# KyleJHarper/tyche

Measured on AMD Instinct MI355X. Metric: GiB/s device-resident LZ4 compress+decompress, 1M×16KiB pages, 1/2/4/8 GPU, higher is better.
Workload: dtype u8

## Files before the change

### tyche_amd/csrc/lz4_encode.hip

```cpp
#include <hip/hip_runtime.h>

#define TYCHE_PHASES_OWNER
#define TYCHE_HASH_LOG 10
#ifndef TYCHE_PARSE_LATCH
#define TYCHE_PARSE_LATCH 1
#endif

#include <algorithm>
#include <cstdlib>

#include "engine.h"
#include "lds_io.h"
#include "lz_parse.h"

namespace tyche {

namespace {

using lzp::kWave;
using lzp::kHashSize;
constexpr uint32_t kPad = 64;
constexpr uint32_t kPrefetchVec = 16;

struct SeqFields {
    uint32_t lit, lext, anchor, off, mc, token, total;
};

__device__ __forceinline__ uint32_t seq_byte(const SeqFields &f, const uint8_t *in, uint32_t rel) {
    const uint32_t lb = 1 + f.lext, ob = lb + f.lit;
    const uint32_t li = f.anchor + min(rel - lb, f.lit - 1u);
    const uint32_t litb = in[rel >= lb && f.lit ? li : 0u];
    const uint32_t ext = rel == f.lext ? (f.lit - 15u) % 255u : 255u;
    const uint32_t mext = rel == f.total - 1u ? (f.mc - 15u) % 255u : 255u;
    uint32_t v = mext;
    v = rel == ob + 1u ? f.off >> 8 : v;
    v = rel == ob ? f.off & 0xFFu : v;
    v = rel < ob ? litb : v;
    v = rel <= f.lext ? ext : v;
    v = rel == 0u ? f.token : v;
    return v;
}


__device__ bool emit_records(const uint2 *rec, uint32_t n, uint32_t anchor, const uint8_t *in, uint8_t *dst,
                             uint32_t &op, uint32_t cap, uint8_t *map, uint4 *fld, uint32_t lane) {
    const bool is_sel = lane < n;
    const uint2 r = rec[is_sel ? lane : 0];
    const uint2 rp = rec[lane > 0 && is_sel ? lane - 1 : 0];
    const uint32_t pos = r.x & 0xFFFFu, cand = r.x >> 16, len = r.y & 0xFFFFu, back = lzp::back_at(in, pos, cand);
    const uint32_t prev_end = lane == 0 ? anchor : (rp.x & 0xFFFFu) + (rp.y & 0xFFFFu);
    SeqFields f{};
    uint32_t enc = 0;
    if (is_sel) {
        const uint32_t k = min(min(back, pos - prev_end), cand);
        f.anchor = prev_end;
        f.lit = pos - k - prev_end;
        f.lext = f.lit >= 15 ? (f.lit - 15) / 255 + 1 : 0;
        f.off = pos - cand;
        f.mc = len + k - kMinMatch;
        const uint32_t mext = f.mc >= 15 ? (f.mc - 15) / 255 + 1 : 0;
        f.token = (min(f.lit, 15u) << 4) | min(f.mc, 15u);
        f.total = 1 + f.lext + f.lit + 2 + mext;
        enc = f.total;
    }
    const int32_t incl = wave_incl_sum((int32_t)enc);
    const uint32_t eo = (uint32_t)incl - enc;
    const uint32_t et = rdlane((uint32_t)incl, 63);
    if (op + et > cap) return false;
    if (is_sel) fld[lane] = make_uint4(f.lit | (f.lext << 16), f.anchor | (f.off << 16), f.mc | (f.total << 16),
                                       eo | (f.token << 16));
    uint32_t *map32 = (uint32_t *)map;
    for (uint32_t j0 = 0; j0 < ((TYCHE_EABLATE & 1) ? 0u : et); j0 += 4u * kWave) {
        const uint64_t before = __ballot(is_sel && eo < j0);
        const int32_t owner0 = before ? 63 - (int32_t)__builtin_clzll(before) : 0;
        map32[lane] = 0xFFFFFFFFu;
        __builtin_amdgcn_wave_barrier();
        if (is_sel && eo >= j0 && eo < j0 + 4u * kWave) map[eo - j0] = (uint8_t)lane;
        __builtin_amdgcn_wave_barrier();
        const uint32_t m = map32[lane];
        int32_t last = -1;
#pragma unroll
        for (int t = 0; t < 4; t++) {
            const uint32_t st = (m >> (8 * t)) & 0xFFu;
            if (st != 0xFFu) last = (int32_t)st;
        }
        const int32_t incl_max = wave_incl_max(last);
        int32_t cur = (int32_t)__shfl(incl_max, (int)(lane ? lane - 1u : 0u));
        cur = max(lane ? cur : -1, owner0);
        const uint32_t jb = j0 + 4u * lane;
        uint32_t word = 0, prev_o = 0xFFFFFFFFu;
        uint4 g = make_uint4(0, 0, 0, 0);
#pragma unroll
        for (int t = 0; t < 4; t++) {
            const uint32_t st = (m >> (8 * t)) & 0xFFu;
            if (st != 0xFFu) cur = (int32_t)st;
            if (jb + (uint32_t)t < et) {
                if ((uint32_t)cur != prev_o) {
                    g = fld[cur];
                    prev_o = (uint32_t)cur;
                }
                SeqFields q;
                q.lit = g.x & 0xFFFFu;
                q.lext = g.x >> 16;
                q.anchor = g.y & 0xFFFFu;
                q.off = g.y >> 16;
                q.mc = g.z & 0xFFFFu;
                q.total = g.z >> 16;
                q.token = g.w >> 16;
                word |= seq_byte(q, in, jb + (uint32_t)t - (g.w & 0xFFFFu)) << (8 * t);
            }
        }
        if (jb + 4u <= et) {
            store_u32_unaligned(dst + op + jb, word);
        } else {
#pragma unroll
            for (int t = 0; t < 4; t++)
                if (jb + (uint32_t)t < et) dst[op + jb + (uint32_t)t] = (uint8_t)(word >> (8 * t));
        }
        __builtin_amdgcn_wave_barrier();
    }
    op += et;
    return true;
}

constexpr uint32_t kOutRing = 512;
constexpr uint32_t kFlushStep = 4u * kWave;
static_assert(kOutRing % kFlushStep == 0 && (kOutRing & (kOutRing - 1)) == 0, "ring");
static_assert(kOutRing + 64u * 8u == 1024u, "emit_records' fields fit the records and the ring");
constexpr uint32_t kLitLane = 8;
struct OutRing {
    uint32_t head, pend;
};

__device__ __forceinline__ void out_flush_steps(const uint8_t *ring, OutRing &r, uint8_t *dst, uint32_t &op,
                                                uint32_t lane) {
    while (r.pend >= kFlushStep) {
        const uint8_t *src = ring + ((r.head + 4u * lane) & (kOutRing - 1));
        store_u32_unaligned(dst + op + 4u * lane, *(const uint32_t *)src);
        op += kFlushStep;
        r.head = (r.head + kFlushStep) & (kOutRing - 1);
        r.pend -= kFlushStep;
    }
}

__device__ __forceinline__ void out_flush_all(const uint8_t *ring, OutRing &r, uint8_t *dst, uint32_t &op,
                                              uint32_t lane) {
    out_flush_steps(ring, r, dst, op, lane);
    for (uint32_t j = 4 * lane; j < r.pend; j += 4 * kWave) {
        const uint32_t w = *(const uint32_t *)(ring + ((r.head + j) & (kOutRing - 1)));
        if (j + 4 <= r.pend) {
            store_u32_unaligned(dst + op + j, w);
        } else {
            for (uint32_t t = 0; j + t < r.pend; t++) dst[op + j + t] = (uint8_t)(w >> (8 * t));
        }
    }
    op += r.pend;
    r.head = 0;
    r.pend = 0;
    __builtin_amdgcn_wave_barrier();
}

__device__ __forceinline__ bool emit_staged(const uint2 *rec, uint32_t n, uint32_t anchor, const uint8_t *in, uint8_t *dst,
                            uint32_t &op, uint32_t cap, uint8_t *ring, OutRing &r, uint8_t *map, uint32_t lane) {
#if defined(TYCHE_PHASES)
    const bool sp_rec = blockIdx.x % 64u == 0u && lane == 0u;
    uint32_t sp_t = (uint32_t)__builtin_amdgcn_s_memtime();
#define SINK_PHASE(i) do { const uint32_t t_ = (uint32_t)__builtin_amdgcn_s_memtime(); \
                           if (sp_rec) atomicAdd(&lzp::g_phase[i], (unsigned long long)(t_ - sp_t)); sp_t = t_; } while (0)
#else
#define SINK_PHASE(i) do {} while (0)
#endif
    const bool is_sel = lane < n;
    const uint2 rc = rec[is_sel ? lane : 0];
    const uint2 rp = rec[lane > 0 && is_sel ? lane - 1 : 0];
    const uint32_t pos = rc.x & 0xFFFFu, cand = rc.x >> 16, len = rc.y & 0xFFFFu, back = lzp::back_at(in, pos, cand);
    const uint32_t prev_end = lane == 0 ? anchor : (rp.x & 0xFFFFu) + (rp.y & 0xFFFFu);
    const uint32_t k = min(min(back, pos - prev_end), cand);
    const uint32_t lstart = prev_end;
    const uint32_t lit = is_sel ? pos - k - prev_end : 0u;
    const uint32_t lext = lit >= 15 ? (lit - 15) / 255 + 1 : 0;
    const uint32_t off = pos - cand;
    const uint32_t mc = len + k - kMinMatch;
    const uint32_t mext = mc >= 15 ? (mc - 15) / 255 + 1 : 0;
    const uint32_t token = (min(lit, 15u) << 4) | min(mc, 15u);
    const uint32_t enc = is_sel ? 1 + lext + lit + 2 + mext : 0u;
    const int32_t incl = wave_incl_sum((int32_t)enc);
    const uint32_t eo = (uint32_t)incl - enc;
    const uint32_t et = rdlane((uint32_t)incl, 63);
    if (op + r.pend + et > cap) return false;
    if (r.pend + et > kOutRing) {
        out_flush_all(ring, r, dst, op, lane);
        uint4 *fld = (uint4 *)(ring + kOutRing - 1024u);
        return emit_records(rec, n, anchor, in, dst, op, cap, map, fld, lane);
    }
    SINK_PHASE(11);
    constexpr uint32_t m = kOutRing - 1;
    const uint32_t q_lit = r.head + r.pend + eo + 1 + lext;
    if (is_sel) {
        uint32_t q = r.head + r.pend + eo;
        ring[q & m] = (uint8_t)token;
        q++;
        for (uint32_t t = 0; t < lext; t++) ring[(q + t) & m] = (uint8_t)(t + 1 == lext ? (lit - 15) % 255 : 255);
        const uint32_t ls = min(lit, kLitLane);
        static_assert(kLitLane == 8, "two gathered dwords");
        const uint32_t ib = (uint32_t)(uintptr_t)in & 3u;
        const uint32_t *A = (const uint32_t *)(in - ib);
        const uint32_t q0 = lstart + ib, i0 = q0 >> 2, sh = q0 & 3u;
        const uint32_t d0 = A[i0], d1 = A[i0 + 1], d2 = A[i0 + 2];
        const uint32_t w0 = __builtin_amdgcn_alignbyte(d1, d0, sh), w1 = __builtin_amdgcn_alignbyte(d2, d1, sh);
#pragma unroll
        for (uint32_t t = 0; t < 8; t++) {
            uint8_t *bp = t < ls ? ring + ((q_lit + t) & m) : map;
            *bp = (uint8_t)((t < 4 ? w0 : w1) >> (8 * (t & 3u)));
        }
        q = q_lit + lit;
        ring[q & m] = (uint8_t)off;
        ring[(q + 1) & m] = (uint8_t)(off >> 8);
        q += 2;
        for (uint32_t t = 0; t < mext; t++) ring[(q + t) & m] = (uint8_t)(t + 1 == mext ? (mc - 15) % 255 : 255);
    }
    SINK_PHASE(12);
    uint64_t longm = __ballot(is_sel && lit > kLitLane);
    while (longm) {
        const uint32_t k = (uint32_t)__builtin_ctzll(longm);
        longm &= longm - 1;
        const uint32_t kl = rdlane(lit, k) - kLitLane, kq = rdlane(q_lit, k) + kLitLane, ks = rdlane(lstart, k) + kLitLane;
        for (uint32_t i = lane; i < kl; i += kWave) ring[(kq + i) & m] = in[ks + i];
    }
    __builtin_amdgcn_wave_barrier();
    SINK_PHASE(13);
    r.pend += et;
    out_flush_steps(ring, r, dst, op, lane);
    __builtin_amdgcn_wave_barrier();
    SINK_PHASE(14);
#if defined(TYCHE_PHASES)
    if (sp_rec) atomicAdd(&lzp::g_phase[15], 1ull);
#endif
    return true;
}
#undef SINK_PHASE

__device__ __noinline__ bool emit_staged_call(const uint2 *rec, uint32_t n, uint32_t anchor, const uint8_t *in, uint8_t *dst,
                                              uint32_t &op, uint32_t cap, uint8_t *ring, OutRing &r, uint8_t *map,
                                              uint32_t lane) {
    return emit_staged(rec, n, anchor, in, dst, op, cap, ring, r, map, lane);
}

__device__ __forceinline__ bool emit_sink_n(const uint2 *rec, uint32_t n, uint32_t anchor, const uint8_t *in, uint8_t *dst,
                                            uint32_t &op, uint32_t cap, uint8_t *ring, OutRing &r, uint8_t *map,
                                            uint32_t lane) {
    return emit_staged(rec, n, anchor, in, dst, op, cap, ring, r, map, lane);
}

__device__ int32_t encode_page(const uint8_t *in, uint32_t L, uint16_t *table, uint8_t *map, uint2 *rec,
                               uint4 *fld, uint8_t *dst, uint32_t cap, uint32_t lane) {
    uint32_t op = 0;
    OutRing r{0u, 0u};
    uint8_t *ring = (uint8_t *)fld;
    auto sink = [&](const uint2 *rr, uint32_t n, uint32_t anchor) -> bool {
        return emit_staged_call(rr, n, anchor, in, dst, op, cap, ring, r, map, lane);
    };
    const uint32_t anchor = lzp::parse_page(in, L, table, rec, lane, sink);
    if (anchor == 0xFFFFFFFFu) return 0;
    out_flush_all(ring, r, dst, op, lane);
    const uint32_t lit = L - anchor;
    const uint32_t lext = lit >= 15 ? (lit - 15) / 255 + 1 : 0;
    const uint32_t total = 1 + lext + lit;
    if (op + total > cap) return 0;
    for (uint32_t j = lane; j < total; j += kWave) {
        uint32_t v;
        if (j == 0) v = min(lit, 15u) << 4;
        else if (j <= lext) v = j == lext ? (lit - 15) % 255 : 255;
        else v = in[anchor + j - 1 - lext];
        dst[op + j] = (uint8_t)v;
    }
    return (int32_t)(op + total);
}

constexpr uint32_t kSplitMin = 12288;
constexpr uint32_t kSplitAt = 36;
static_assert(kSplitAt >= 32 && kSplitAt < 64, "B's half must fit its scratch (sized for L / 2 + 64)");
constexpr uint32_t kSplitPrefetch = 8;
struct SplitHdr {
    uint32_t next_lo, next_hi, next2_lo, next2_hi;
    uint32_t len_a;
    uint32_t len_b;
    uint32_t has_first;
    int32_t result;
    uint2 first;
    uint32_t pad[6];
};
static_assert(sizeof(SplitHdr) == 64, "split header");
__device__ __forceinline__ void seed_table(const uint8_t *in, uint16_t *table, uint32_t from, uint32_t to,
                                           uint32_t lane) {
    const uint32_t ib = (uint32_t)(uintptr_t)in & 3u;
    const uint32_t la = lzp::lds_addr(in - ib) + ((lane + ib) & ~3u), ls = (lane + ib) & 3u;
    const uint32_t tbase = rfl(lzp::lds_addr(table));
    auto slot = [&](uint32_t w) { return (lzp::lds_u16_t *)(uintptr_t)lzp::slot_addr(tbase, lzp::hash4(w)); };
    uint32_t blk = from;
    for (; blk + 4u * kWave <= to; blk += 4u * kWave) {
        const lzp::lds_u32_t *P = (const lzp::lds_u32_t *)(uintptr_t)(la + blk);
        uint32_t w[4];
#pragma unroll
        for (uint32_t u = 0; u < 4u; u++) w[u] = lzp::word_at(P[16u * u], P[16u * u + 1u], ls);
#pragma unroll
        for (uint32_t u = 0; u < 4u; u++) {
            *slot(w[u]) = (uint16_t)(blk + kWave * u + lane);
            __builtin_amdgcn_wave_barrier();
        }
    }
    for (; blk < to; blk += kWave) {
        const lzp::lds_u32_t *P = (const lzp::lds_u32_t *)(uintptr_t)(la + blk);
        *slot(lzp::word_at(P[0], P[1], ls)) = (uint16_t)(blk + lane);
        __builtin_amdgcn_wave_barrier();
    }
}

constexpr size_t kWaveRegion = kHashSize * sizeof(uint16_t) + 4 * kWave + kWave * sizeof(uint2) + kOutRing;
constexpr size_t kSplitStage = sizeof(SplitHdr) + 2 * kWaveRegion;

__device__ bool write_last_literals(const uint8_t *in, uint32_t anchor, uint32_t L, uint8_t *dst, uint32_t &op,
                                    uint32_t cap, uint32_t lane) {
    const uint32_t lit = L - anchor;
    const uint32_t lext = lit >= 15 ? (lit - 15) / 255 + 1 : 0;
    const uint32_t total = 1 + lext + lit;
    if (op + total > cap) return false;
    for (uint32_t j = lane; j < total; j += kWave) {
        uint32_t v;
        if (j == 0) v = min(lit, 15u) << 4;
        else if (j <= lext) v = j == lext ? (lit - 15) % 255 : 255;
        else v = in[anchor + j - 1 - lext];
        dst[op + j] = (uint8_t)v;
    }
    op += total;
    return true;
}

__device__ __forceinline__ bool emit_joint(uint2 first, uint32_t prev_end, const uint8_t *in, uint8_t *dst, uint32_t &op,
                                           uint32_t cap, uint32_t lane) {
    const uint32_t pos = first.x & 0xFFFFu, cand = first.x >> 16, len = first.y & 0xFFFFu;
    const uint32_t back = rfl(lzp::back_at(in, pos, cand));
    const uint32_t k = min(min(back, pos - prev_end), cand);
    SeqFields f;
    f.anchor = prev_end;
    f.lit = pos - k - prev_end;
    f.lext = f.lit >= 15 ? (f.lit - 15) / 255 + 1 : 0;
    f.off = pos - cand;
    f.mc = len + k - kMinMatch;
    const uint32_t mext = f.mc >= 15 ? (f.mc - 15) / 255 + 1 : 0;
    f.token = (min(f.lit, 15u) << 4) | min(f.mc, 15u);
    f.total = 1 + f.lext + f.lit + 2 + mext;
    if (op + f.total > cap) return false;
    for (uint32_t j = lane; j < f.total; j += kWave) dst[op + j] = (uint8_t)seq_byte(f, in, j);
    op += f.total;
    return true;
}

typedef uint32_t u32x4_ua __attribute__((ext_vector_type(4), aligned(1)));
typedef __attribute__((address_space(1))) u32x4_ua g_u32x4_ua;

__global__ __launch_bounds__(128, 3) void lz4_encode_split_kernel(tyche_batch_t b, uint32_t in_cap, unsigned *ctr,
                                                                   uint8_t *ws, uint32_t ws_stride) {
    extern __shared__ __attribute__((aligned(16))) uint8_t smem[];
    const uint32_t tid = threadIdx.x, lane = tid & 63u;
    const uint32_t wave = rfl(tid >> 6);
    SplitHdr *hdr = (SplitHdr *)smem;
    uint8_t *region = smem + sizeof(SplitHdr) + wave * kWaveRegion;
    uint16_t *table = (uint16_t *)region;
    uint8_t *map = region + kHashSize * sizeof(uint16_t);
    uint2 *rec = (uint2 *)(map + 4 * kWave);
    uint4 *fld = (uint4 *)(rec + kWave);
    uint8_t *ring = (uint8_t *)fld;
    uint8_t *stage = smem + kSplitStage;
    uint8_t *scratch = ws + (size_t)blockIdx.x * ws_stride;

    size_t page = blockIdx.x;
    if (page >= b.count) return;
    PageRef p = batch_page(b, page);
    uint32_t head = stage_in(p.src, p.src_len <= in_cap ? p.src_len : 0, stage, tid, 2 * kWave);
    if (tid == 0) {
        const size_t nx = (size_t)atomicAdd(ctr, 1u) + gridDim.x;
        hdr->next_lo = (uint32_t)nx;
        hdr->next_hi = (uint32_t)(nx >> 32);
    }
    for (;;) {
        for (uint32_t w = lane; w < kHashSize / 8; w += kWave) ((u32x4 *)table)[w] = u32x4{0, 0, 0, 0};
        if (tid < kWave) stage[head + p.src_len + tid] = 0;
        __syncthreads();
        const size_t next = (size_t)rfl(hdr->next_lo) | ((size_t)rfl(hdr->next_hi) << 32);
        PageRef pn;
        TYCHE_NEXT_PAGE(kSplitPrefetch);
        if (next < b.count) {
            pn = batch_page(b, next);
            TYCHE_NEXT_PAGE_FETCH(kSplitPrefetch, 2 * kWave, pn.src, pn.src_len, in_cap, tid)
        }
        const uint8_t *in = stage + head;
        const uint32_t L = p.src_len;
        const bool fits = L <= in_cap;
        const bool split = fits && L >= kSplitMin;
        const uint32_t H = (L * kSplitAt / 64u) & ~(kWave - 1u);
        uint32_t opA = 0, cursorA = 0;
        bool okA = true;
        OutRing rA{0u, 0u};
        int32_t rv = 0;
        if (wave == 0) {
            if (fits && !split) {
                rv = encode_page(in, L, table, map, rec, fld, p.dst, p.dst_cap, lane);
            } else if (split) {
                auto sink = [&](const uint2 *rr, uint32_t n, uint32_t anchor) -> bool {
                    return emit_staged(rr, n, anchor, in, p.dst, opA, p.dst_cap, ring, rA, map, lane);
                };
                cursorA = lzp::parse_page(in, H + kLastLiterals, table, rec, lane, sink);
                okA = cursorA != 0xFFFFFFFFu;
                if (okA) out_flush_all(ring, rA, p.dst, opA, lane);
            }
            if (lane == 0) {
                const size_t nx = (size_t)atomicAdd(ctr, 1u) + gridDim.x;
                hdr->next2_lo = (uint32_t)nx;
                hdr->next2_hi = (uint32_t)(nx >> 32);
            }
        } else if (split) {
            seed_table(in, table, 0u, H, lane);
            uint32_t op = 0;
            OutRing r{0u, 0u};
            bool first = true;
            if (lane == 0) hdr->has_first = 0;
            auto sink = [&](const uint2 *rr, uint32_t n, uint32_t anchor) -> bool {
                if (first) {
                    first = false;
                    if (lane == 0) {
                        hdr->first = rr[0];
                        hdr->has_first = 1;
                    }
                    if (n == 1) return true;
                    const uint32_t a = (rr[0].x & 0xFFFFu) + (rr[0].y & 0xFFFFu);
                    return emit_staged(rr + 1, n - 1, a, in, scratch, op, 0xFFFFFFFFu, ring, r, map, lane);
                }
                return emit_staged(rr, n, anchor, in, scratch, op, 0xFFFFFFFFu, ring, r, map, lane);
            };
            const uint32_t anchor = lzp::parse_page(in, L, table, rec, lane, sink, H);
            out_flush_all(ring, r, scratch, op, lane);
            if (!first) (void)write_last_literals(in, anchor, L, scratch, op, 0xFFFFFFFFu, lane);
            if (lane == 0) hdr->len_b = first ? 0u : op;
        }
        __syncthreads();
        if (wave == 0) {
            if (!fits) {
                rv = kResultTooLarge;
            } else if (split) {
                rv = 0;
                if (okA) {
                    const uint32_t lb = rfl(hdr->len_b);
                    bool ok;
                    if (rfl(hdr->has_first)) {
                        if (lane == 0) rec[0] = hdr->first;
                        __builtin_amdgcn_wave_barrier();
                        ok = emit_staged(rec, 1, cursorA, in, p.dst, opA, p.dst_cap, ring, rA, map, lane);
                        if (ok) out_flush_all(ring, rA, p.dst, opA, lane);
                    } else {
                        ok = write_last_literals(in, cursorA, L, p.dst, opA, p.dst_cap, lane);
                    }
                    if (ok && (uint64_t)opA + lb <= p.dst_cap) rv = (int32_t)(opA + lb);
                }
                if (lane == 0) hdr->len_a = opA;
            }
            if (lane == 0) {
                hdr->result = rv;
                b.results[page] = rv;
            }
        }
        __syncthreads();
        if (split) {
            const int32_t res = (int32_t)rfl((uint32_t)hdr->result);
            const uint32_t la = rfl(hdr->len_a), lb = rfl(hdr->len_b);
            if (res > 0 && lb) {
                uint8_t *d = p.dst + la;
                const uint32_t nv = lb >> 4;
                for (uint32_t v = tid; v < nv; v += 2 * kWave)
                    *(g_u32x4_ua *)(uintptr_t)(d + 16 * v) = gload_nt((const u32x4 *)(scratch + 16 * v));
                for (uint32_t j = (nv << 4) + tid; j < lb; j += 2 * kWave) d[j] = scratch[j];
            }
        }
        __syncthreads();
        if (next >= b.count) break;
        page = next;
        p = pn;
        head = nhead;
        TYCHE_NEXT_PAGE_INSTALL(kSplitPrefetch, 2 * kWave, p.src, p.src_len, in_cap, stage, tid)
        if (tid == 0) {
            hdr->next_lo = hdr->next2_lo;
            hdr->next_hi = hdr->next2_hi;
        }
    }
}

constexpr uint32_t kSeed = 4096;
template <uint32_t kNW>
struct SplitHdrN {
    uint32_t next_lo, next_hi, next2_lo, next2_hi;
    int32_t result;
    uint32_t pad0[3];
    uint32_t len[kNW];
    uint32_t cursor[kNW];
    uint32_t has_first[kNW];
    uint32_t ok[kNW];
    uint32_t seg[kNW];
    uint2 first[kNW];
};
template <uint32_t kNW>
constexpr size_t split_hdr_bytes() { return (sizeof(SplitHdrN<kNW>) + 63) & ~(size_t)63; }
template <uint32_t kNW>
constexpr size_t split_stage_off() { return split_hdr_bytes<kNW>() + kNW * kWaveRegion; }
template <uint32_t kNW>
__host__ __device__ constexpr uint32_t part_scratch(uint32_t in_cap) {
    return (lz4_bound(in_cap / kNW + 2u * kWave) + 64u + 255u) & ~255u;
}
template <uint32_t kNW>
constexpr uint32_t split_prefetch() { return (16384u / 16u + kNW * kWave - 1u) / (kNW * kWave); }

template <uint32_t kNW, bool kRagged>
__global__ __launch_bounds__(kNW * 64) __attribute__((amdgpu_waves_per_eu(5))) void lz4_encode_splitn_kernel(
    tyche_batch_t b, uint32_t in_cap, unsigned *ctr, uint8_t *ws, uint32_t ws_stride, uint32_t seed, uint32_t p0) {
    extern __shared__ __attribute__((aligned(16))) uint8_t smem[];
    constexpr uint32_t kT = kNW * kWave;
    constexpr uint32_t kPf = split_prefetch<kNW>();
    const uint32_t tid = threadIdx.x, lane = tid & 63u;
    const uint32_t wave = rfl(tid >> 6);
    SplitHdrN<kNW> *hdr = (SplitHdrN<kNW> *)smem;
    uint8_t *region = smem + split_hdr_bytes<kNW>() + wave * kWaveRegion;
    uint16_t *table = (uint16_t *)region;
    uint8_t *map = region + kHashSize * sizeof(uint16_t);
    uint2 *rec = (uint2 *)(map + 4 * kWave);
    uint4 *fld = (uint4 *)(rec + kWave);
    uint8_t *ring = (uint8_t *)fld;
    uint8_t *stage = smem + split_stage_off<kNW>();
    const uint32_t part_ws = part_scratch<kNW>(in_cap);
    uint8_t *scratch = ws + (size_t)blockIdx.x * ws_stride + (size_t)(wave ? wave - 1u : 0u) * part_ws;

    size_t page = blockIdx.x;
    if (page >= b.count) return;
    PageRef p = batch_page(b, page);
    uint32_t head = stage_in(p.src, p.src_len <= in_cap ? p.src_len : 0, stage, tid, kT);
    if (tid == 0) {
        const size_t nx = (size_t)atomicAdd(ctr, 1u) + gridDim.x;
        hdr->next_lo = (uint32_t)nx;
        hdr->next_hi = (uint32_t)(nx >> 32);
    }
    for (;;) {
        for (uint32_t w = lane; w < kHashSize / 8; w += kWave) ((u32x4 *)table)[w] = u32x4{0, 0, 0, 0};
        if (tid < kWave) stage[head + p.src_len + tid] = 0;
        __syncthreads();
        const size_t next = (size_t)rfl(hdr->next_lo) | ((size_t)rfl(hdr->next_hi) << 32);
        PageRef pn;
        TYCHE_NEXT_PAGE(kPf);
        if (next < b.count) {
            pn = batch_page(b, next);
            TYCHE_NEXT_PAGE_FETCH(kPf, kT, pn.src, pn.src_len, in_cap, tid)
        }
        const uint8_t *in = stage + head;
        const uint32_t L = p.src_len;
        const bool fits = L <= in_cap;
        auto bnd = [&](uint32_t w) -> uint32_t {
            if (w == 0) return 0u;
            if (w == kNW) return L;
            if (!p0) return ((L * w) / kNW) & ~(kWave - 1u);
            const uint32_t h = (L * p0 / 64u) & ~(kWave - 1u);
            return (h + ((L - h) * (w - 1u)) / (kNW - 1u)) & ~(kWave - 1u);
        };
        const uint32_t b0 = bnd(wave);
        const uint32_t b1 = bnd(wave + 1);
        const uint32_t Lp = wave + 1 == kNW ? L : b1 + kLastLiterals;
        if (fits) {
            if (wave > 0) {
                seed_table(in, table, b0 > seed ? b0 - seed : 0u, b0, lane);
                if (lane == 0) hdr->has_first[wave] = 0;
            }
            uint8_t *odst = wave == 0 ? p.dst : scratch;
            const uint32_t ocap = wave == 0 ? p.dst_cap : 0xFFFFFFFFu;
            uint32_t op = 0;
            OutRing r{0u, 0u};
            bool first = wave > 0;
            auto sink = [&](const uint2 *rr, uint32_t n, uint32_t anchor) -> bool {
                const uint2 *r2 = rr;
                uint32_t n2 = n, a2 = anchor;
                if (first) {
                    first = false;
                    if (lane == 0) {
                        hdr->first[wave] = rr[0];
                        hdr->has_first[wave] = 1;
                    }
                    r2 = rr + 1;
                    n2 = n - 1;
                    a2 = (rr[0].x & 0xFFFFu) + (rr[0].y & 0xFFFFu);
                    if (n2 == 0) return true;
                }
                return emit_sink_n(r2, n2, a2, in, odst, op, ocap, ring, r, map, lane);
            };
            const uint32_t cur = lzp::parse_page(in, Lp, table, rec, lane, sink, b0);
            if (wave == 0) {
                const bool ok = cur != 0xFFFFFFFFu;
                if (ok) out_flush_all(ring, r, p.dst, op, lane);
                if (lane == 0) {
                    hdr->ok[0] = ok ? 1u : 0u;
                    hdr->len[0] = op;
                    hdr->cursor[0] = ok ? cur : 0u;
                    const size_t nx = (size_t)atomicAdd(ctr, 1u) + gridDim.x;
                    hdr->next2_lo = (uint32_t)nx;
                    hdr->next2_hi = (uint32_t)(nx >> 32);
                }
            } else {
                const bool had = !first;
                out_flush_all(ring, r, scratch, op, lane);
                if (had && wave + 1 == kNW) (void)write_last_literals(in, cur, L, scratch, op, 0xFFFFFFFFu, lane);
                if (lane == 0) {
                    hdr->len[wave] = had ? op : 0u;
                    hdr->cursor[wave] = cur;
                }
            }
        } else if (kRagged && tid == 0) {
            const size_t nx = (size_t)atomicAdd(ctr, 1u) + gridDim.x;
            hdr->next2_lo = (uint32_t)nx;
            hdr->next2_hi = (uint32_t)(nx >> 32);
        }
        __syncthreads();
        if (wave == 0) {
            int32_t rv = 0;
            if (!fits) {
                rv = kResultTooLarge;
            } else if (rfl(hdr->ok[0])) {
                uint32_t op = rfl(hdr->len[0]), cur = rfl(hdr->cursor[0]);
                bool ok = true, tail_done = false;
                for (uint32_t w = 1; w < kNW && ok; w++) {
                    if (!rfl(hdr->has_first[w])) {
                        if (lane == 0) hdr->seg[w] = op;
                        continue;
                    }
                    const uint2 fr = hdr->first[w];
                    ok = emit_joint(make_uint2(rfl(fr.x), rfl(fr.y)), cur, in, p.dst, op, p.dst_cap, lane);
                    if (lane == 0) hdr->seg[w] = op;
                    op += rfl(hdr->len[w]);
                    cur = rfl(hdr->cursor[w]);
                    tail_done = w + 1 == kNW;
                }
                if (ok && !tail_done) ok = write_last_literals(in, cur, L, p.dst, op, p.dst_cap, lane);
                if (ok && op <= p.dst_cap) rv = (int32_t)op;
            }
            if (lane == 0) {
                hdr->result = rv;
                b.results[page] = rv;
            }
        }
        __syncthreads();
        if (wave > 0 && fits) {
            const int32_t res = (int32_t)rfl((uint32_t)hdr->result);
            const uint32_t lw = rfl(hdr->len[wave]);
            if (res > 0 && lw) {
                uint8_t *d = p.dst + rfl(hdr->seg[wave]);
                const uint32_t nv = lw >> 4;
                for (uint32_t v = lane; v < nv; v += kWave)
                    *(g_u32x4_ua *)(uintptr_t)(d + 16 * v) = gload_nt((const u32x4 *)(scratch + 16 * v));
                for (uint32_t j = (nv << 4) + lane; j < lw; j += kWave) d[j] = scratch[j];
            }
        }
        __syncthreads();
        if (next >= b.count) break;
        page = next;
        p = pn;
        head = nhead;
        TYCHE_NEXT_PAGE_INSTALL(kPf, kT, p.src, p.src_len, in_cap, stage, tid)
        if (tid == 0) {
            hdr->next_lo = hdr->next2_lo;
            hdr->next_hi = hdr->next2_hi;
        }
    }
}

__global__ __launch_bounds__(64) void lz4_encode_kernel(tyche_batch_t b, uint32_t in_cap, unsigned *ctr) {
    extern __shared__ __attribute__((aligned(16))) uint8_t smem[];
    const uint32_t lane = threadIdx.x;
    uint16_t *table = (uint16_t *)smem;
    uint8_t *map = smem + kHashSize * sizeof(uint16_t);
    uint2 *rec = (uint2 *)(map + 4 * kWave);
    uint4 *fld = (uint4 *)(rec + kWave);
    uint8_t *stage = (uint8_t *)fld + kOutRing;
    const size_t stride = gridDim.x;

    size_t page = blockIdx.x;
    if (page >= b.count) return;
    PageRef p = batch_page(b, page);
    uint32_t head = stage_in(p.src, p.src_len <= in_cap ? p.src_len : 0, stage, lane, kWave);
    for (;;) {
        const size_t next = ctr ? claim_page(ctr, lane) : page + stride;
        PageRef pn;
        TYCHE_NEXT_PAGE(kPrefetchVec);
        if (next < b.count) {
            pn = batch_page(b, next);
            TYCHE_NEXT_PAGE_FETCH(kPrefetchVec, kWave, pn.src, pn.src_len, in_cap, lane)
        }
        int32_t rv;
        if (p.src_len > in_cap) {
            rv = kResultTooLarge;
        } else {
            uint8_t *in = stage + head;
            for (uint32_t w = lane; w < kHashSize / 8; w += kWave) ((u32x4 *)table)[w] = u32x4{0, 0, 0, 0};
            WAVE_SYNC();
            in[p.src_len + lane] = 0;
            WAVE_SYNC();
            rv = encode_page(in, p.src_len, table, map, rec, fld, p.dst, p.dst_cap, lane);
        }
        if (lane == 0) b.results[page] = rv;
        if (next >= b.count) break;
        WAVE_SYNC();
        page = next;
        p = pn;
        head = nhead;
        TYCHE_NEXT_PAGE_INSTALL(kPrefetchVec, kWave, p.src, p.src_len, in_cap, stage, lane)
    }
}

}

hipError_t launch_lz4_encode(const tyche_batch_t &b, uint32_t in_cap, hipStream_t s) {
    if (b.count == 0) return hipSuccess;
    if (in_cap > 65535u) {
        if (in_cap > TYCHE_LZ4_MAX_PAGE || knob("LZ4_EXACT", 0) != 0) return hipErrorInvalidValue;
        if (b.src_lengths) {
            const hipError_t e = launch_lz4_encode(b, 65535u, s);
            if (e != hipSuccess) return e;
        }
        return launch_lz4_encode_large(b, in_cap, b.src_lengths ? 65536u : 0u, s);
    }
    if (knob("LZ4_EXACT", 0) != 0) return launch_lz4_encode_exact(b, in_cap, s);
    if (knob("LZ4_HC", 0) != 0) return launch_lz4_encode_hc(b, in_cap, s);
    const bool one_wave = knob("LZ4_ENC", 0) == 1;
    const long nw = knob("LZ4_ENC_WAVES", 4);
    const uint32_t split_min = (uint32_t)std::max(0L, knob("LZ4_SPLIT_MIN", nw == 3 || nw == 4 || nw == 8 ? 8192L
                                                                                                       : (long)kSplitMin));
    if (!one_wave && in_cap >= split_min && (nw == 3 || nw == 4 || nw == 8)) {
        const bool rg = b.src_lengths != nullptr;
        const void *k = nw == 8   ? (rg ? (const void *)lz4_encode_splitn_kernel<8, true> : (const void *)lz4_encode_splitn_kernel<8, false>)
                        : nw == 4 ? (rg ? (const void *)lz4_encode_splitn_kernel<4, true> : (const void *)lz4_encode_splitn_kernel<4, false>)
                                  : (rg ? (const void *)lz4_encode_splitn_kernel<3, true> : (const void *)lz4_encode_splitn_kernel<3, false>);
        const uint32_t T = (uint32_t)nw * kWave;
        const size_t lds = (nw == 8 ? split_stage_off<8>() : nw == 4 ? split_stage_off<4>() : split_stage_off<3>()) +
                           ((in_cap + 16u + kPad + 15u) & ~15u);
        const size_t grid = page_grid(k, T, lds, b.count, "LZ4_ENC_PAGES_PER_CU");
        const uint32_t pws = nw == 8 ? part_scratch<8>(in_cap) : nw == 4 ? part_scratch<4>(in_cap) : part_scratch<3>(in_cap);
        uint32_t seed = (uint32_t)std::max(0L, knob("LZ4_ENC_SEED", nw == 3 ? 10240L : nw == 4 ? 8192L : (long)kSeed)) &
                        ~(kWave - 1u);
        uint32_t p0 = (uint32_t)std::max(0L, knob("LZ4_ENC_P0", nw == 3 ? 27L : nw == 4 ? 19L : 0L));
        if (p0) p0 = std::min<uint32_t>(std::max<uint32_t>(p0, (64u + (uint32_t)nw - 1u) / (uint32_t)nw), 48u);
        const uint32_t ws_stride = (uint32_t)(nw - 1) * pws;
        ScratchLease ws(s, grid * (size_t)ws_stride);
        if (ws.get()) {
            WorkCounter ctr(s, grid < b.count);
            if (!ctr.get()) return hipErrorOutOfMemory;
            unsigned *cp = ctr.get();
            uint8_t *wp = (uint8_t *)ws.get();
            void *args[] = {(void *)&b, &in_cap, &cp, &wp, (void *)&ws_stride, &seed, &p0};
            (void)hipLaunchKernel(k, dim3((unsigned)grid), dim3(T), args, lds, s);
            return hipGetLastError();
        }
    }
    if (!one_wave && in_cap >= split_min) {
        const size_t lds = kSplitStage + ((in_cap + 16u + kPad + 15u) & ~15u);
        const size_t grid = page_grid((const void *)lz4_encode_split_kernel, 2 * kWave, lds, b.count);
        const uint32_t ws_stride = (lz4_bound(in_cap / 2u + kWave) + 64u + 255u) & ~255u;
        ScratchLease ws(s, grid * (size_t)ws_stride);
        if (ws.get()) {
            WorkCounter ctr(s, grid < b.count);
            if (!ctr.get()) return hipErrorOutOfMemory;
            hipLaunchKernelGGL(lz4_encode_split_kernel, dim3((unsigned)grid), dim3(2 * kWave), lds, s, b, in_cap,
                               ctr.get(), (uint8_t *)ws.get(), ws_stride);
            return hipGetLastError();
        }
    }
    const size_t lds = kHashSize * sizeof(uint16_t) + 4 * kWave + kWave * 8 + kOutRing +
                       ((in_cap + 16u + kPad + 15u) & ~15u);
    const size_t grid = page_grid((const void *)lz4_encode_kernel, kWave, lds, b.count);
    WorkCounter ctr(s, grid < b.count);
    if (!ctr.get()) return hipErrorOutOfMemory;
    hipLaunchKernelGGL(lz4_encode_kernel, dim3((unsigned)grid), dim3(kWave), lds, s, b, in_cap, ctr.get());
    return hipGetLastError();
}

#ifdef TYCHE_PHASES
extern "C" int tyche_phase_read(unsigned long long *out) {
    if (hipMemcpyFromSymbol(out, HIP_SYMBOL(lzp::g_phase), 16 * sizeof(unsigned long long)) != hipSuccess) return -1;
    static const unsigned long long zero[16] = {};
    return hipMemcpyToSymbol(HIP_SYMBOL(lzp::g_phase), zero, sizeof(zero)) == hipSuccess ? 0 : -1;
}
#endif

}
```

Baseline: 205.3.

## Reuse the previous wave's hash table to cut redundant seed hashing in split encoder

In the multi-wave split LZ4 encoder, each wave after the first used to rehash a seed window of up to `seed` bytes before its boundary. Now, when that window reaches back past the previous wave's start, a wave seeds only from the previous boundary. It then merges entries from the previous wave's LDS hash table, keeping positions at or after the seed start. This removes redundant hashing but adds LDS flag handshakes between neighbouring waves, using spin-waits with sleep and a timeout that reports a sync-failure result. It risks serialising the waves and adds a new failure code.

```diff
diff --git a/tyche_amd/csrc/lz4_encode.hip b/tyche_amd/csrc/lz4_encode.hip
--- a/tyche_amd/csrc/lz4_encode.hip
+++ b/tyche_amd/csrc/lz4_encode.hip
@@ -499,7 +499,10 @@
 struct SplitHdrN {
     uint32_t next_lo, next_hi, next2_lo, next2_hi;
     int32_t result;
-    uint32_t pad0[3];
+    uint32_t sync_fail;
+    uint32_t pad0[2];
+    uint32_t seeded[kNW];
+    uint32_t taken[kNW];
     uint32_t len[kNW];
     uint32_t cursor[kNW];
     uint32_t has_first[kNW];
@@ -518,9 +521,40 @@
 template <uint32_t kNW>
 constexpr uint32_t split_prefetch() { return (16384u / 16u + kNW * kWave - 1u) / (kNW * kWave); }
 
+constexpr int32_t kResultSeedSync = INT32_MIN + 1;
+constexpr uint32_t kSeedWaitPolls = 1u << 22;
+typedef __attribute__((address_space(3))) uint32_t lds_flag_t;
+__device__ __forceinline__ void flag_set(uint32_t *flag, uint32_t turn, uint32_t lane) {
+    if (lane == 0) __hip_atomic_store((lds_flag_t *)(uintptr_t)lzp::lds_addr(flag), turn, __ATOMIC_RELEASE, __HIP_MEMORY_SCOPE_WORKGROUP);
+}
+__device__ __forceinline__ bool flag_wait(uint32_t *flag, uint32_t turn) {
+    lds_flag_t *f = (lds_flag_t *)(uintptr_t)lzp::lds_addr(flag);
+    for (uint32_t i = 0; i < kSeedWaitPolls; i++) {
+        if (rfl(__hip_atomic_load(f, __ATOMIC_ACQUIRE, __HIP_MEMORY_SCOPE_WORKGROUP)) == turn) return true;
+        __builtin_amdgcn_s_sleep(2);
+    }
+    return false;
+}
+__device__ __forceinline__ uint32_t merge_slots(uint32_t mine, uint32_t prev, uint32_t s) {
+    const uint32_t pl = prev & 0xFFFFu, ph = prev >> 16;
+    const uint32_t lo = (mine & 0xFFFFu) ? (mine & 0xFFFFu) : pl >= s ? pl : 0u;
+    const uint32_t hi = (mine >> 16) ? (mine >> 16) : ph >= s ? ph : 0u;
+    return lo | (hi << 16);
+}
+__device__ __forceinline__ void merge_table(uint16_t *table, const uint16_t *prev, uint32_t s, uint32_t lane) {
+    static_assert(kHashSize % (8 * kWave) == 0, "16-byte vectors over the lanes");
+#pragma unroll
+    for (uint32_t v = lane; v < kHashSize / 8; v += kWave) {
+        const u32x4 m = ((const u32x4 *)table)[v], q = ((const u32x4 *)prev)[v];
+        ((u32x4 *)table)[v] = u32x4{merge_slots(m.x, q.x, s), merge_slots(m.y, q.y, s), merge_slots(m.z, q.z, s),
+                                    merge_slots(m.w, q.w, s)};
+    }
+}
+
 template <uint32_t kNW, bool kRagged>
 __global__ __launch_bounds__(kNW * 64) __attribute__((amdgpu_waves_per_eu(5))) void lz4_encode_splitn_kernel(
-    tyche_batch_t b, uint32_t in_cap, unsigned *ctr, uint8_t *ws, uint32_t ws_stride, uint32_t seed, uint32_t p0) {
+    tyche_batch_t b, uint32_t in_cap, unsigned *ctr, uint8_t *ws, uint32_t ws_stride, uint32_t seed, uint32_t p0,
+    uint32_t merge) {
     extern __shared__ __attribute__((aligned(16))) uint8_t smem[];
     constexpr uint32_t kT = kNW * kWave;
     constexpr uint32_t kPf = split_prefetch<kNW>();
@@ -546,7 +580,14 @@
         hdr->next_lo = (uint32_t)nx;
         hdr->next_hi = (uint32_t)(nx >> 32);
     }
+    if (tid < kNW) {
+        hdr->seeded[tid] = 0;
+        hdr->taken[tid] = 0;
+        hdr->sync_fail = 0;
+    }
+    uint32_t turn = 0;
     for (;;) {
+        turn++;
         for (uint32_t w = lane; w < kHashSize / 8; w += kWave) ((u32x4 *)table)[w] = u32x4{0, 0, 0, 0};
         if (tid < kWave) stage[head + p.src_len + tid] = 0;
         __syncthreads();
@@ -572,7 +613,26 @@
         const uint32_t Lp = wave + 1 == kNW ? L : b1 + kLastLiterals;
         if (fits) {
             if (wave > 0) {
-                seed_table(in, table, b0 > seed ? b0 - seed : 0u, b0, lane);
+                const uint32_t s0 = b0 > seed ? b0 - seed : 0u;
+                if (!merge) {
+                    seed_table(in, table, s0, b0, lane);
+                } else {
+                    const uint32_t bp = bnd(wave - 1u);
+                    const bool mg = wave >= 2u && s0 < bp;
+                    bool ok = true;
+                    if (wave >= 2u && !mg) flag_set(&hdr->taken[wave - 1u], turn, lane);
+                    seed_table(in, table, mg ? bp : s0, b0, lane);
+                    if (mg) {
+                        ok = flag_wait(&hdr->seeded[wave - 1u], turn);
+                        merge_table(table, (const uint16_t *)(region - kWaveRegion), s0, lane);
+                        flag_set(&hdr->taken[wave - 1u], turn, lane);
+                    }
+                    if (wave + 1u < kNW) {
+                        flag_set(&hdr->seeded[wave], turn, lane);
+                        ok = flag_wait(&hdr->taken[wave], turn) && ok;
+                    }
+                    if (!ok && lane == 0) hdr->sync_fail = turn;
+                }
                 if (lane == 0) hdr->has_first[wave] = 0;
             }
             uint8_t *odst = wave == 0 ? p.dst : scratch;
@@ -627,6 +687,8 @@
             int32_t rv = 0;
             if (!fits) {
                 rv = kResultTooLarge;
+            } else if (rfl(hdr->sync_fail) == turn) {
+                rv = kResultSeedSync;
             } else if (rfl(hdr->ok[0])) {
                 uint32_t op = rfl(hdr->len[0]), cur = rfl(hdr->cursor[0]);
                 bool ok = true, tail_done = false;
@@ -750,6 +812,7 @@
                         ~(kWave - 1u);
         uint32_t p0 = (uint32_t)std::max(0L, knob("LZ4_ENC_P0", nw == 3 ? 27L : nw == 4 ? 19L : 0L));
         if (p0) p0 = std::min<uint32_t>(std::max<uint32_t>(p0, (64u + (uint32_t)nw - 1u) / (uint32_t)nw), 48u);
+        uint32_t merge = knob("LZ4_ENC_SEED_MERGE", 1) != 0 ? 1u : 0u;
         const uint32_t ws_stride = (uint32_t)(nw - 1) * pws;
         ScratchLease ws(s, grid * (size_t)ws_stride);
         if (ws.get()) {
@@ -757,7 +820,7 @@
             if (!ctr.get()) return hipErrorOutOfMemory;
             unsigned *cp = ctr.get();
             uint8_t *wp = (uint8_t *)ws.get();
-            void *args[] = {(void *)&b, &in_cap, &cp, &wp, (void *)&ws_stride, &seed, &p0};
+            void *args[] = {(void *)&b, &in_cap, &cp, &wp, (void *)&ws_stride, &seed, &p0, &merge};
             (void)hipLaunchKernel(k, dim3((unsigned)grid), dim3(T), args, lds, s);
             return hipGetLastError();
         }
```

Result: no change. 206.5 (median of 6 runs) (+0.6%).
